# google-research/robopianist

Measured on AMD Instinct MI355X. Metric: env-steps/sec (whole node) at 4096 envs/GPU, higher is better.
Workload: dtype f64

## Files before the change

### include/rp_engine.h

```cpp
#ifndef RP_ENGINE_H
#define RP_ENGINE_H

#include <stddef.h>
#include <stdint.h>

#ifdef __cplusplus
extern "C" {
#endif

typedef struct rp_engine rp_engine;

typedef enum {
  RP_QPOS = 0,
  RP_QVEL = 1,
  RP_QACC_WARMSTART = 2,
  RP_CTRL = 3,
  RP_QFRC_APPLIED = 4,
  RP_ACT_FORCE = 5,
  RP_ACT_VELOCITY = 6,
  RP_SITE_XPOS = 7,
  RP_TIME = 8,
  RP_NCON = 9,
  RP_CONTACT_GEOMS = 10,
  RP_WARN_FLAGS = 11,
// ... 18 lines not shown
#define RP_WARN_SPLIT_FULL 64
#define RP_WARN_DENSE_FULL 32

int rp_create(const void* model_blob, size_t blob_bytes, int n_envs, int device_id,
              int precision, rp_engine** out);
int rp_destroy(rp_engine* e);

int rp_reset(rp_engine* e, const uint8_t* mask);

int rp_set(rp_engine* e, rp_field f, const void* src);
int rp_get(rp_engine* e, rp_field f, void* dst);

int rp_step(rp_engine* e, int n_substeps, uint32_t* key_trace);

int rp_forward(rp_engine* e);

int rp_step_masked(rp_engine* e, int n_substeps, uint32_t* key_trace, const uint8_t* reset_mask);

int rp_set_solver_limits(rp_engine* e, int max_newton_iter, int max_ls_iter);

int rp_set_solver_tolerance(rp_engine* e, double tolerance, double ls_tolerance);
int rp_set_mpr_tolerance(rp_engine* e, double tolerance, double polytope_tolerance);
int rp_set_lazy_position_stage(rp_engine* e, int on);
int rp_set_legacy_step(rp_engine* e, int on);
int rp_set_cost_ordered_launch(rp_engine* e, int on);
int rp_set_lean_solver(rp_engine* e, int on);

int rp_set_fused_substeps(rp_engine* e, int on);
int rp_get_fused_substeps(rp_engine* e);

int rp_set_split_position_stage(rp_engine* e, int on);
int rp_get_split_position_stage(rp_engine* e);

int rp_set_stream_slices(rp_engine* e, int n);
int rp_set_acc_sensors(rp_engine* e, int on);
int rp_sync(rp_engine* e);
int rp_get_stream(rp_engine* e, void** hip_stream);
int rp_set_stream(rp_engine* e, void* hip_stream);
int rp_field_ptr(rp_engine* e, rp_field f, void** ptr, size_t* bytes);
int rp_n_envs(const rp_engine* e);
int rp_dim(const rp_engine* e, const char* name);
int rp_kernel_time(rp_engine* e, double* avg_ms, int* n_launches);
int rp_solver_kernel_time(rp_engine* e, double* avg_ms, int* n_launches);
int rp_solver_kernel_envs(rp_engine* e, double* avg_envs);
int rp_solver_kernel_fused(rp_engine* e);
int rp_profile(rp_engine* e, long long* out, int n, int enable);
// ... 7 lines not shown
```

### robopianist_amd/csrc/rp_engine.hip

```cpp
#include "rp_kernels.hpp"
#include "rp_schedule.hpp"

#include <hip/hip_runtime.h>

#include <cmath>
#include <cstdio>
#include <cstdlib>
#include <cstring>
#include <map>
#include <mutex>
#include <string>
#include <vector>

#include "../../include/rp_engine.h"

namespace {

__global__ void rp_lead_mask_kernel(int* lead, const int* active, const unsigned char* valid, int lazy, const unsigned char* also, int n) {
  const int e = blockIdx.x * blockDim.x + threadIdx.x;
  if (e < n) lead[e] = (((active ? active[e] != 0 : true) && !(lazy && valid[e])) || (also && also[e])) ? 1 : 0;
}
__global__ void rp_mark_valid_kernel(unsigned char* valid, const int* active, const unsigned char* also, int n) {
  const int e = blockIdx.x * blockDim.x + threadIdx.x;
  if (e < n && (!active || active[e] != 0 || (also && also[e]))) valid[e] = 1;
}

#define RP_ORDER_BUCKETS 256
#define RP_ORDER_CLASSES 8
__global__ __launch_bounds__(512) void rp_order_kernel(int* order_all, const int* hdr, const int* active, int base, int n,
                                                       int* heavy_list, int* heavy_cnt, unsigned char* listed) {
  const int x = blockIdx.x;
  if (heavy_list) {
    for (int e = x + RP_ORDER_CLASSES * (int)threadIdx.x; e < n; e += RP_ORDER_CLASSES * blockDim.x) {
      const bool on = hdr[(base + e) * rpk::HDR_N + rpk::HDR_CLASS] != 1 && !(active && active[base + e] == 0);
      if (on) heavy_list[base + atomicAdd(heavy_cnt, 1)] = base + e;
      if (listed) listed[base + e] = on ? 1 : 0;
    }
  }
  if (!order_all) return;
  int* order = order_all + base;
  __shared__ int hist[RP_ORDER_BUCKETS];
  for (int i = threadIdx.x; i < RP_ORDER_BUCKETS; i += blockDim.x) hist[i] = 0;
  __syncthreads();
// ... 202 lines not shown
    if (!ev_pending[i]) return;
    if (wait) hipEventSynchronize(ev1[i]);
    else if (hipEventQuery(ev1[i]) != hipSuccess) return;
    float ms = 0;
    if (hipEventElapsedTime(&ms, ev0[i], ev1[i]) == hipSuccess) {
      kernel_ms += ms; kernel_launches++;
    }
    if (sv_envs[i] > 0 && hipEventElapsedTime(&ms, sv0[i], sv1[i]) == hipSuccess) {
      const int kd = sv_kind[i] & 1;
      solver_ms_k[kd] += ms; solver_launches_k[kd]++; solver_envs_k[kd] += sv_envs[i];
    }
    sv_envs[i] = 0;
    ev_pending[i] = false;
  }
  virtual int reset(const uint8_t* mask) = 0;
  virtual int set(rp_field f, const void* src) = 0;
  virtual int get(rp_field f, void* dst) = 0;
  virtual int step(int nsub, uint32_t* trace, int mode, const uint8_t* reset_mask = nullptr) = 0;
  virtual void limits(int newton, int ls) = 0;
  virtual void tolerances(double tol, double ls_tol) = 0;
  virtual void mpr_tolerances(double tol, double poly_tol) = 0;
  bool lazy_position = false;
  bool legacy_step = true;
  bool cost_order = false;
  int n_slices = 1;
  static const int kMaxSlices = kRpMaxSlices;
  hipStream_t xstream[kMaxSlices] = {};
  hipEvent_t ev_fork = nullptr, ev_join[kMaxSlices] = {};
  hipStream_t hstream[kMaxSlices] = {};
  hipEvent_t ev_hfork[kMaxSlices] = {}, ev_hjoin[kMaxSlices] = {};
  virtual int acc_sensors(int on) = 0;
  virtual int lean_solver(int on) = 0;
  virtual int fused_substeps(int on) = 0;
  virtual int fused_substeps_on() const = 0;
  virtual int split_position(int on) = 0;
  virtual int split_position_on() const = 0;
  virtual int field_ptr(rp_field f, void** p, size_t* bytes) = 0;
  bool own_stream = true;
  virtual int profile(long long* out, int n, int enable) = 0;
};

template <typename T>
struct Engine : EngineBase {
  RpModel<T> M{};
  RpState<T> S{};
  RpStage<T> B{};
// ... 242 lines not shown
    hipMemset(B.slots, 0xFF, sizeof(int) * E * rpk::SLOT_N);
    hipMemset(B.keyslot, 0xFF, sizeof(int) * E * (RPK_NKEYS / 4));
    S.key_trace = nullptr;
    S.prof = nullptr;
    d_active = dalloc<int>(E);
    S.active = nullptr;
    d_lead = dalloc<int>(E);
    d_order = dalloc<int>(E);
    {
      std::vector<int> id(E);
      for (size_t i = 0; i < E; i++) id[i] = (int)i;
      hipMemcpy(d_order, id.data(), E * sizeof(int), hipMemcpyHostToDevice);
    }
    S.cost_pos = dalloc<int>(E); S.cost_sol = dalloc<int>(E);
    d_heavy = dalloc<int>(E); d_heavy_cnt = dalloc<int>(2 * kMaxSlices);
    d_listed = dalloc<unsigned char>(E); S.listed = d_listed;
    d_heavy_peak = dalloc<int>(kMaxSlices + 1);
    if (hipHostMalloc((void**)&h_heavy_peak, sizeof(int) * (kMaxSlices + 1)) != hipSuccess) { (void)hipGetLastError(); h_heavy_peak = nullptr; }
    else { for (int i = 0; i < kMaxSlices; i++) h_heavy_peak[i] = -1; h_heavy_peak[kMaxSlices] = 0; }
    S.heavy_list = nullptr; S.heavy_cnt = nullptr; S.heavy_done = nullptr;
    S.qpos_prev = nullptr; S.qvel_prev = nullptr;
    d_valid = dalloc<unsigned char>(E);
    S.max_newton = M.iterations; S.max_ls = M.ls_iterations;
  }
  void read_switches() {
    {
      const char* sp = getenv("RP_SPLIT_POS");
      split_capable = sizeof(T) == 8 && !deep;
      split_mode = !split_capable ? 0 : (sp ? (sp[0] == '0' ? 0 : (sp[0] == '1' ? 1 : 2)) : 2);
    }
    {
      const char* le = getenv("RP_LEAN");
      lean = sizeof(T) == 8 && !deep && !(le && le[0] == '0');
      const char* dh = getenv("RP_DENSE_HANDS");
      dense_joint = (dh && dh[0] == '0') ? RPK_LEAN_JOINT : 0;
      S.lean = lean ? (1 | dense_joint) : 0;
      if (lean && le && atoi(le) > 1) S.lean = (atoi(le) & RPK_LEAN_CAP) | dense_joint;
    }
  }

  bool split_alloc_failed = false;
  bool ensure_split_buffers() {
    if (B.frames) return true;
    if (split_alloc_failed) return false;
    const size_t E = (size_t)nenv;
    const size_t mark = allocs.size();
    try {
      T* frames = dalloc<T>(E * RPK_NFRAME * 64);
      B.cand = dalloc<int>(E * RPK_NCAND * 2);
      B.ncand = dalloc<int>(E);
      B.cres = dalloc<T>(E * RPK_NRES * 12);
      B.cres_n = dalloc<int>(E * RPK_NCAND);
// ... 104 lines not shown
    if (newton > 0) S.max_newton = newton;
    if (ls > 0) S.max_ls = ls;
  }

  RpState<T> reset_state() const {
    RpState<T> sr = S;
    sr.sens_torque = sensors_on ? d_sens_torque : nullptr; sr.sens_touch = sensors_on ? d_sens_touch : nullptr;
    return sr;
  }
  RpState<T> heavy_state(const RpState<T>& ss, int sl, bool capturing) const {
    RpState<T> sh = ss;
    sh.heavy_list = d_heavy + ss.env_base; sh.heavy_cnt = d_heavy_cnt + 2 * sl; sh.heavy_done = d_heavy_cnt + 2 * sl + 1;
    sh.heavy_peak = capturing ? nullptr : d_heavy_peak + sl;
    return sh;
  }
  RpState<T> sensor_state(const RpState<T>& ss) const {
    RpState<T> sq = ss;
    sq.qpos = d_qpos_prev; sq.qvel = d_qvel_prev;
    sq.sens_torque = d_sens_torque; sq.sens_touch = d_sens_touch;
    sq.key_trace = nullptr; sq.prof = nullptr;
    return sq;
  }

  void launch_reset(const unsigned char* dmask) {
    hipLaunchKernelGGL(rp_reset_kernel<T>, dim3(nenv), dim3(64), 0, stream, reset_state(), d_qpos0, dmask, nv, nu, nsite, d_valid);
  }
  int reset(const uint8_t* mask) override {
    HIP_OK(hipSetDevice(device));
    const unsigned char* dmask = nullptr;
    if (mask) {
      if (is_device_ptr(mask)) dmask = mask;
      else {
        if (!d_mask) HIP_OK(hipMalloc((void**)&d_mask, (size_t)nenv));
        HIP_OK(hipMemcpyAsync(d_mask, mask, (size_t)nenv, hipMemcpyHostToDevice, stream));
        HIP_OK(hipStreamSynchronize(stream));
        dmask = d_mask;
      }
    }
    launch_reset(dmask);
    HIP_OK(hipGetLastError());
    return 0;
  }

  bool field(rp_field f, void** p, size_t* bytes, bool* writable) {
    size_t E = (size_t)nenv;
    *writable = false;
    switch (f) {
      case RP_QPOS: *p = S.qpos; *bytes = sizeof(T) * E * nv; *writable = true; return true;
      case RP_QVEL: *p = S.qvel; *bytes = sizeof(T) * E * nv; *writable = true; return true;
      case RP_QACC_WARMSTART: *p = S.warm; *bytes = sizeof(T) * E * nv; *writable = true; return true;
      case RP_CTRL: *p = S.ctrl; *bytes = sizeof(T) * E * nu; *writable = true; return true;
      case RP_QFRC_APPLIED: *p = S.qfrc_applied; *bytes = sizeof(T) * E * nv; *writable = true; return true;
      case RP_ACT_FORCE: *p = S.act_force; *bytes = sizeof(T) * E * nu; return true;
      case RP_ACT_VELOCITY: *p = S.act_vel; *bytes = sizeof(T) * E * nu; return true;
      case RP_SITE_XPOS: *p = S.site_xpos; *bytes = sizeof(T) * E * nsite * 3; return true;
      case RP_TIME: *p = S.time; *bytes = sizeof(T) * E; *writable = true; return true;
      case RP_NCON: *p = S.ncon; *bytes = sizeof(int) * E; return true;
      case RP_CONTACT_GEOMS: *p = S.contact_geoms; *bytes = sizeof(int) * E * RPK_NCOUT * 2; return true;
      case RP_WARN_FLAGS: *p = S.warn; *bytes = sizeof(int) * E; *writable = true; return true;
      case RP_SOLVER_ITER: *p = S.solver_iter; *bytes = sizeof(int) * E; return true;
      case RP_CONTACT_DIST: *p = S.contact_dist; *bytes = sizeof(T) * E * RPK_NCOUT; return true;
      case RP_ACTIVE: *p = d_active; *bytes = sizeof(int) * E; *writable = true; return true;
// ... 3 lines not shown
      case RP_DEBUG_HANDOVER_HDR: *p = B.hdr; *bytes = sizeof(int) * E * rpk::HDR_N; return true;
      case RP_SENSOR_TORQUE: if (!d_sens_torque) return false; *p = d_sens_torque; *bytes = sizeof(T) * E * nv; return true;
      case RP_SENSOR_TOUCH: if (!d_sens_touch) return false; *p = d_sens_touch; *bytes = sizeof(T) * E * nsite; return true;
    }
    return false;
  }
  int field_ptr(rp_field f, void** p, size_t* bytes) override {
    bool w;
    if (!field(f, p, bytes, &w)) return fail("rp_field_ptr: unknown field (sensor fields need rp_set_acc_sensors first)");
    if (f == RP_ACTIVE) S.active = d_active;
    return 0;
  }
  int set(rp_field f, const void* src) override {
    void* p; size_t nb; bool w;
    if (!field(f, &p, &nb, &w)) return fail("rp_set: unknown field");
    if (!w) return fail("rp_set: field is read-only");
    if (!src) { if (f == RP_ACTIVE) { S.active = nullptr; return 0; } return fail("rp_set: null source"); }
    HIP_OK(hipSetDevice(device));
    if (nb) {
      if (!is_device_ptr(src)) HIP_OK(hipStreamSynchronize(stream));
      HIP_OK(hipMemcpyAsync(p, src, nb, hipMemcpyDefault, stream));
    }
    if (f == RP_ACTIVE) S.active = d_active;
    if (f == RP_QPOS || f == RP_QVEL || f == RP_TREE_OFFSET) HIP_OK(hipMemsetAsync(d_valid, 0, (size_t)nenv, stream));
    return 0;
  }
  int get(rp_field f, void* dst) override {
    void* p; size_t nb; bool w;
    if (!field(f, &p, &nb, &w)) return fail("rp_get: unknown field");
    if (!dst) return fail("rp_get: null destination");
    HIP_OK(hipSetDevice(device));
    if (nb) HIP_OK(hipMemcpyAsync(dst, p, nb, hipMemcpyDefault, stream));
    if (!is_device_ptr(dst)) HIP_OK(hipStreamSynchronize(stream));
    return 0;
  }

  struct StepCtx {
    int nsub = 0, mode = 0;
    const uint8_t* reset_mask = nullptr;
    bool capturing = false, timeit = false, lead_masked = false;
    int slot = 0;
    RpStepInput in;
    RpStepPlan plan;
    int nsl = 1;
    RpState<T> s;
  };
  struct Slice {
// ... 152 lines not shown
      HIP_OK(hipEventRecord(ev_hjoin[sl], hs));
      RpState<T> sm_ = x.ss;
      sm_.skip_heavy = 1;
      emit_pos(c, x, sm_, k);
      HIP_OK(hipStreamWaitEvent(st, ev_hjoin[sl], 0));
    } else {
      emit_pos(c, x, x.ss, k);
    }
    return 0;
  }

  int finish(const StepCtx& c, uint32_t* trace, size_t trace_words) {
    HIP_OK(hipGetLastError());
    if (c.mode == 0) step_calls++;
    if (c.timeit) { HIP_OK(hipEventRecord(ev1[c.slot], stream)); ev_pending[c.slot] = true; }
    if (trace && c.mode == 0)
      HIP_OK(hipMemcpyAsync(trace, d_trace, trace_words * sizeof(uint32_t), hipMemcpyDefault, stream));
    return 0;
  }

  int step(int nsub, uint32_t* trace, int mode, const uint8_t* reset_mask = nullptr) override {
    HIP_OK(hipSetDevice(device));
    if (mode == 0 && nsub <= 0) return fail("rp_step: n_substeps must be positive");
    if (reset_mask) {
      if (!is_device_ptr(reset_mask)) return fail("rp_step_masked: the reset mask must be device memory");
      launch_reset(reset_mask);
    }
    StepCtx c;
    c.nsub = nsub; c.mode = mode; c.reset_mask = reset_mask;
    c.s = S;
    const size_t need = (size_t)nenv * (nsub > 0 ? nsub : 1) * 4;
    if (trace && mode == 0) {
      if (need > trace_cap) {
        if (d_trace) hipFree(d_trace);
        HIP_OK(hipMalloc((void**)&d_trace, need * sizeof(uint32_t)));
        trace_cap = need;
      }
      c.s.key_trace = d_trace;
    }
    RP_TRY(begin_timers(c));
    plan(c);
    if (cost_order && mode == 0) c.s.order = d_order;
    const bool lazy_now = lazy_position && legacy_step;
    c.s.stale_outputs = (!legacy_step && mode == 0) ? 1 : 0;
    c.lead_masked = (lazy_now || reset_mask) && mode == 0;
    if (c.lead_masked)
      hipLaunchKernelGGL(rp_lead_mask_kernel, dim3((nenv + 255) / 256), dim3(256), 0, stream, d_lead, c.s.active, d_valid, lazy_now ? 1 : 0, reset_mask, nenv);
    RP_TRY(fork_slices(c));
    for (int sl = 0; sl < c.nsl; sl++) {
      Slice x = slice_of(c, sl);
      RpState<T> lead = x.ss;
      lead.order = nullptr;
      if (c.lead_masked) lead.active = d_lead;
      emit_pos(c, x, lead, -1);
      if (mode != 0) continue;
      if (c.plan.fused_now && sizeof(T) == 8) { RP_TRY(emit_fused_slice(c, x)); continue; }
      for (int k = 0; k < nsub; k++) RP_TRY(emit_substep(c, x, k));
    }
    RP_TRY(join_slices(c));
    return finish(c, trace, need);
  }
};

EngineBase* E(rp_engine* e) { return reinterpret_cast<EngineBase*>(e); }

}

extern "C" {

const char* rp_last_error(void) { return g_err.c_str(); }

int rp_create(const void* model_blob, size_t blob_bytes, int n_envs, int device_id, int precision,
              rp_engine** out) {
  if (!out) return fail("rp_create: out is null");
  *out = nullptr;
  if (!model_blob || n_envs <= 0) return fail("rp_create: bad arguments");
  if (precision != 32 && precision != 64) return fail("rp_create: precision must be 32 or 64");
  Blob b;
  if (!b.init(model_blob, blob_bytes)) return fail("rp_create: not a model blob (bad magic)");
  if (!b.has("eng_nlink")) return fail("rp_create: blob lacks engine tables (eng_*)");
  int ndev = 0;
  if (hipGetDeviceCount(&ndev) != hipSuccess || ndev <= 0)
// ... 20 lines not shown
  if (r) { delete e; return r; }
  *out = reinterpret_cast<rp_engine*>(e);
  return 0;
}

int rp_destroy(rp_engine* e) {
  if (!e) return fail("rp_destroy: null engine");
  delete E(e);
  return 0;
}
int rp_reset(rp_engine* e, const uint8_t* mask) { return e ? E(e)->reset(mask) : fail("null engine"); }
int rp_set(rp_engine* e, rp_field f, const void* src) { return e ? E(e)->set(f, src) : fail("null engine"); }
int rp_get(rp_engine* e, rp_field f, void* dst) { return e ? E(e)->get(f, dst) : fail("null engine"); }
int rp_step(rp_engine* e, int n_substeps, uint32_t* key_trace) {
  return e ? E(e)->step(n_substeps, key_trace, 0) : fail("null engine");
}
int rp_forward(rp_engine* e) { return e ? E(e)->step(0, nullptr, 1) : fail("null engine"); }
int rp_step_masked(rp_engine* e, int n_substeps, uint32_t* key_trace, const uint8_t* reset_mask) {
  return e ? E(e)->step(n_substeps, key_trace, 0, reset_mask) : fail("null engine");
}
int rp_set_solver_limits(rp_engine* e, int max_newton_iter, int max_ls_iter) {
  if (!e) return fail("null engine");
  E(e)->limits(max_newton_iter, max_ls_iter);
  return 0;
}
int rp_profile(rp_engine* e, long long* out, int n, int enable) {
  return e ? E(e)->profile(out, n, enable) : fail("null engine");
}
int rp_set_mpr_tolerance(rp_engine* e, double tolerance, double polytope_tolerance) {
  if (!e) return fail("null engine");
  E(e)->mpr_tolerances(tolerance, polytope_tolerance);
  return 0;
}
int rp_set_solver_tolerance(rp_engine* e, double tolerance, double ls_tolerance) {
  if (!e) return fail("null engine");
  E(e)->tolerances(tolerance, ls_tolerance);
  return 0;
}
int rp_set_lazy_position_stage(rp_engine* e, int on) {
  if (!e) return fail("null engine");
  E(e)->lazy_position = on != 0;
  return 0;
}
int rp_set_legacy_step(rp_engine* e, int on) {
  if (!e) return fail("null engine");
  E(e)->legacy_step = on != 0;
  return 0;
}
int rp_set_acc_sensors(rp_engine* e, int on) { return e ? E(e)->acc_sensors(on) : fail("null engine"); }
int rp_set_lean_solver(rp_engine* e, int on) { return e ? E(e)->lean_solver(on) : fail("null engine"); }
int rp_set_fused_substeps(rp_engine* e, int on) { return e ? E(e)->fused_substeps(on) : fail("null engine"); }
int rp_get_fused_substeps(rp_engine* e) { return e ? E(e)->fused_substeps_on() : fail("null engine"); }
int rp_set_split_position_stage(rp_engine* e, int on) { return e ? E(e)->split_position(on) : fail("null engine"); }
int rp_get_split_position_stage(rp_engine* e) { return e ? E(e)->split_position_on() : fail("null engine"); }
int rp_set_stream_slices(rp_engine* e, int n) {
  if (!e) return fail("null engine");
  if (n != 0 && n != 1 && n != 2 && n != 3 && n != 4) return fail("rp_set_stream_slices: 0 (automatic), 1, 2, 3 or 4");
  E(e)->n_slices = n;
  return 0;
}
int rp_set_cost_ordered_launch(rp_engine* e, int on) {
  if (!e) return fail("null engine");
  E(e)->cost_order = on != 0;
  return 0;
}
int rp_sync(rp_engine* e) {
  if (!e) return fail("null engine");
  HIP_OK(hipSetDevice(E(e)->device));
  HIP_OK(hipStreamSynchronize(E(e)->stream));
  return 0;
}
int rp_set_stream(rp_engine* e, void* hip_stream) {
  if (!e) return fail("null engine");
  EngineBase* b = E(e);
  HIP_OK(hipSetDevice(b->device));
  HIP_OK(hipStreamSynchronize(b->stream));
  for (int i = 0; i < EngineBase::kRing; i++) b->harvest(i, true);
  if (b->own_stream && b->stream) HIP_OK(hipStreamDestroy(b->stream));
  b->stream = (hipStream_t)hip_stream;
  b->own_stream = false;
  return 0;
}
int rp_field_ptr(rp_engine* e, rp_field f, void** ptr, size_t* bytes) {
  if (!e || !ptr || !bytes) return fail("null argument");
  return E(e)->field_ptr(f, ptr, bytes);
}
// ... 55 lines not shown
```

### robopianist_amd/csrc/rp_kernels.hpp

```cpp
#pragma once
#include <type_traits>
#include "rp_model.hpp"
#include "rp_wave.hpp"
#include "rp_narrow.hpp"
#include "rp_collide.hpp"
#include "rp_dense.hpp"
#include "rp_solver2.hpp"
#include "rp_solver_full.hpp"

#define RPK_BOXBOX(rc_, bx_, pA_, mA_, sA_, pB_, mB_, sB_) [&]() -> int {                       \
    T a_[15], b_[15]; RawCon<T> o_[3];                                                          \
    _Pragma("unroll") for (int i_ = 0; i_ < 3; i_++) { a_[i_] = (pA_)[i_]; b_[i_] = (pB_)[i_]; a_[12 + i_] = (sA_)[i_]; b_[12 + i_] = (sB_)[i_]; } \
    _Pragma("unroll") for (int i_ = 0; i_ < 9; i_++) { a_[3 + i_] = (mA_)[i_]; b_[3 + i_] = (mB_)[i_]; }                     \
    const int n_ = box_box(o_, bx_, a_, a_ + 3, a_ + 12, b_, b_ + 3, b_ + 12);                  \
    (rc_)[0] = o_[0]; (rc_)[1] = o_[1]; (rc_)[2] = o_[2];                                       \
    return n_; }()
namespace rpk {
template <typename T, int MD>
struct Smem<T, 0, MD> : SmemShared<T> {
  T xpos[RPK_NLX(MD)][3];
  T xmat[RPK_NLX(MD)][9];
  T xaxis[RPK_NLX(MD)][3];
  T xanchor[RPK_NLX(MD)][3];
  union {
// ... 38 lines not shown
      unsigned short glist[RPK_GLIST];
      unsigned short klist[RPK_KLIST];
    };
  };
  union {
    T acc[RPK_NLX(MD)][10];
    struct {
      float gax[RPK_WAVE][4];
      float grr[RPK_WAVE];
      int clist[RPK_NCAND];
    };
  };
  T gpos[RPK_WAVE][3];
};
template <typename T, int MD>
struct Smem<T, 2, MD> : Smem<T, 0, MD> {
  T fext[RPK_NLX(MD)][6];
  T touch[RPK_WAVE];
};
}

template <typename T>
__global__ void rp_reset_kernel(RpState<T> S, const T* qpos0, const unsigned char* mask, int nv, int nu, int nsite,
                                unsigned char* stage_valid) {
  const int env = blockIdx.x;
  if (mask && !mask[env]) return;
  if (threadIdx.x == 0) stage_valid[env] = 0;
  for (int i = threadIdx.x; i < nv; i += blockDim.x) {
    S.qpos[(size_t)env * nv + i] = qpos0[i];
    S.qvel[(size_t)env * nv + i] = 0;
    S.warm[(size_t)env * nv + i] = 0;
    S.qfrc_applied[(size_t)env * nv + i] = 0;
  }
  for (int i = threadIdx.x; i < nu; i += blockDim.x) S.ctrl[(size_t)env * nu + i] = 0;
  if (threadIdx.x == 0) { S.time[env] = 0; S.warn[env] = 0; }
  if (S.sens_torque) for (int i = threadIdx.x; i < nv; i += blockDim.x) S.sens_torque[(size_t)env * nv + i] = 0;
  if (S.sens_touch) for (int i = threadIdx.x; i < nsite; i += blockDim.x) S.sens_touch[(size_t)env * nsite + i] = 0;
}

template <typename T, int MODE, int MD = RPK_MAXD, int MESH = 0, bool EXT = false, int PART = 0>
__device__ __forceinline__ void rp_position_body(const RpModel<T>& M, const RpState<T>& S, const RpStage<T>& B, const int substep,
                                                 const int nsub, const int env, void* ext, const int lane) {
  static_assert(MODE == 0 || MODE == 2, "position / velocity stage (0) or sensor stage (2)");
  using namespace rpk;
  using N = Num<T>;
  constexpr bool PB = MODE == 0 && PART == 2 && !EXT;
  constexpr bool PF = MODE == 0 && PART == 1 && !EXT;
  if constexpr (MODE == 0) {
    if constexpr (PART == 2) { if constexpr (!PB) { if (B.ncand[env] < 0) return; } }
    else if (S.skip_heavy && S.listed[env]) return;
  }
  const int env_active = S.active ? S.active[env] : 1;
  using SM_ = std::conditional_t<(MODE == 0 && PART == 1), SmemFront<T, MD>, Smem<T, MODE, MD>>;
  SM_& sm = rp_smem<SM_, EXT>(ext);
#ifdef RPK_POISON_LDS
  {
    unsigned* w_ = reinterpret_cast<unsigned*>(&sm);
    for (int i = threadIdx.x; i < (int)(sizeof(sm) / 4); i += 64) w_[i] = 0xFFF4DEADu;
// ... 1881 lines not shown
```

### robopianist_amd/csrc/rp_model.hpp

```cpp
#pragma once
#include <hip/hip_runtime.h>
#include <stdint.h>

#define RPK_WAVE 64
#define RPK_NC 64
#define RPK_NCOUT 64
#ifndef RPK_NCL
#define RPK_NCL 32
#endif
#ifndef RPK_NE
#define RPK_NE 640
#endif
#define RPK_EM0(lane_, con_, col_, cross_) ((lane_) | ((con_) << 6) | ((col_) << 12) | ((cross_) << 16))
#define RPK_EM1(base_, cnt_, rank_) ((base_) | ((cnt_) << 12) | ((rank_) << 18))
#define RPK_EM_LANE(m0_) ((m0_) & 63)
#define RPK_EM_CON(m0_) (((m0_) >> 6) & 63)
#define RPK_EM_COL(m0_) (((m0_) >> 12) & 15)
#define RPK_EM_CROSS(m0_) (((m0_) >> 16) & 1)
#define RPK_EM_BASE(m1_) ((m1_) & 4095)
#define RPK_EM_CNT(m1_) (((m1_) >> 12) & 63)
#define RPK_EM_RANK(m1_) (((m1_) >> 18) & 63)
#define RPK_NBOXF 32
#ifndef RPK_HMAX
#define RPK_HMAX 60
// ... 271 lines not shown
template <typename T>
struct RpStage {
  T* RM;
  T* lanef;
  int* lanei;
  int* hdr;
  T* entJ;
  int* entM;
  int* slots;
  int* keyslot;
  T* covf;
  int* covi;
  T* frames;
  int* cand;
  int* ncand;
  T* cres;
  int* cres_n;
  int* tlist;
  int* tcount;
  int tcount_off;
  size_t tstride;
  int* split_dropped;
};
```

### robopianist_amd/csrc/rp_schedule.hpp

```cpp
#pragma once

static const int kRpMaxSlices = 4;

struct RpStepInput {
  int nenv = 0;
  int mode = 0;
  int n_slices = 1;
  int fused = 2;
  bool fused_capable = false;
  int split_mode = 0;
  bool split_capable = false;
  bool split_dropped = false;
  bool capturing = false;
  bool lean = false, deep = false, graph = false;
  double heavy_est[kRpMaxSlices] = {8, 8, 8, 8};
  int last_nsl = 1;
  bool many_heavy = false;
};

struct RpStepPlan {
  int sched = 0;
  int nsl = 1;
  bool fused_now = false;
  bool split_wanted = false;
// ... 30 lines not shown
    else if (split_ok && !p.many_heavy) p.sched = 4;
    else p.sched = in.nenv >= kRpNoSlicesFrom ? 1 : 2;
    p.fused_now = p.sched == 3;
    want = p.sched == 2 ? 2 : (p.sched == 4 ? 3 : 1);
    sched4 = p.sched == 4;
  }
  p.split_wanted = in.split_capable && in.mode == 0 && (in.split_mode == 1 || sched4);
  p.nsl = (in.mode == 0 && want > 1 && in.nenv >= kRpSliceMinEnvs && !in.capturing && !p.fused_now) ? (want >= 4 ? 4 : want) : 1;
  p.companion_now = p.nsl <= 2;
  return p;
}

inline int rp_fused_report(const RpStepInput& in, int auto_mode) {
  return !in.fused_capable ? 0 : (in.fused == 1 ? 1 : (in.fused == 2 && in.n_slices == 0 ? (auto_mode == 3 ? 1 : 2) : 0));
}
inline int rp_split_report(const RpStepInput& in, int auto_mode) {
  return in.split_mode == 1 ? 1 : (in.split_mode == 2 && in.n_slices == 0 && in.nenv >= kRpFusedBelow && !in.split_dropped ? (auto_mode == 4 ? 1 : 2) : 0);
}

inline bool rp_heavy_pos_alongside(const RpStepInput& in, bool on_companion_stream, bool fp64, double est) {
  return on_companion_stream && !in.deep && !in.graph && fp64 && est >= kRpHeavyOn;
}

inline int rp_slice_bound(int nenv, int nsl, int sl) { return sl >= nsl ? nenv : (int)(((long long)nenv * sl / nsl + 7) / 8 * 8); }

inline int rp_order_threads_for(int cnt) {
  const int t = ((cnt / 16 + 63) / 64) * 64;
  return t < 64 ? 64 : (t > 512 ? 512 : t);
}

inline double rp_heavy_est_update(double est, int seen) { return seen > est ? seen : 0.9 * est + 0.1 * seen; }

inline int rp_heavy_grid(double est, int cnt, int max_grid) {
  int g = (int)(2.0 * est) + 2;
  g = g < 2 ? 2 : (g > max_grid ? max_grid : g);
  return cnt < g ? cnt : g;
}
```

### robopianist_amd/engine.py

```python

from __future__ import annotations

import ctypes
import os
from typing import Optional

import numpy as np

from robopianist_amd import _abi
from robopianist_amd.model import compile as mcompile
from robopianist_amd.model import engine_tables

_HERE = os.path.dirname(os.path.abspath(__file__))
LIB_PATH = os.environ.get("RP_ENGINE_LIB") or os.path.join(_HERE, "csrc", "librp_engine.so")

QPOS, QVEL, QACC_WARMSTART, CTRL, QFRC_APPLIED, ACT_FORCE, ACT_VELOCITY, SITE_XPOS, \
    TIME, NCON, CONTACT_GEOMS, WARN_FLAGS, SOLVER_ITER, CONTACT_DIST, TREE_OFFSET, ACTIVE, \
    SENSOR_TORQUE, SENSOR_TOUCH, ENV_COST, DEBUG_MASS_ROWS, DEBUG_HANDOVER_HDR = range(21)
MAX_CONTACTS = 64

WARN_BADSTATE = 1
WARN_CONTACT_FULL = 2
WARN_HESSIAN = 4
WARN_KEYSLOT_FULL = 8
WARN_WORK_FULL = 16
WARN_SPLIT_FULL = 64
WARN_DENSE_FULL = 32

EXPORTED_SYMBOLS = (
    "rp_create", "rp_destroy", "rp_reset", "rp_set", "rp_get", "rp_step", "rp_forward", "rp_step_masked",
    "rp_set_solver_limits", "rp_set_solver_tolerance", "rp_set_mpr_tolerance", "rp_set_lazy_position_stage", "rp_set_legacy_step", "rp_set_cost_ordered_launch", "rp_set_stream_slices", "rp_set_lean_solver", "rp_set_fused_substeps", "rp_get_fused_substeps", "rp_set_split_position_stage", "rp_get_split_position_stage", "rp_set_acc_sensors", "rp_sync", "rp_get_stream", "rp_set_stream", "rp_field_ptr",
    "rp_n_envs", "rp_dim",
    "rp_kernel_time", "rp_solver_kernel_time", "rp_solver_kernel_envs", "rp_solver_kernel_fused", "rp_profile", "rp_last_error",
)

_lib = None


class EngineError(RuntimeError):
    pass


def load_library(path: str = LIB_PATH):
    global _lib
    if _lib is not None:
        return _lib
    L = _abi.open_library(path, "engine", EngineError)
    L.rp_last_error.restype = ctypes.c_char_p
    L.rp_create.argtypes = [ctypes.c_char_p, ctypes.c_size_t, ctypes.c_int, ctypes.c_int,
                            ctypes.c_int, ctypes.POINTER(ctypes.c_void_p)]
    L.rp_destroy.argtypes = [ctypes.c_void_p]
    L.rp_reset.argtypes = [ctypes.c_void_p, ctypes.c_void_p]
    L.rp_set.argtypes = [ctypes.c_void_p, ctypes.c_int, ctypes.c_void_p]
    L.rp_get.argtypes = [ctypes.c_void_p, ctypes.c_int, ctypes.c_void_p]
    L.rp_step.argtypes = [ctypes.c_void_p, ctypes.c_int, ctypes.c_void_p]
    L.rp_forward.argtypes = [ctypes.c_void_p]
    L.rp_step_masked.argtypes = [ctypes.c_void_p, ctypes.c_int, ctypes.c_void_p, ctypes.c_void_p]
    L.rp_set_solver_limits.argtypes = [ctypes.c_void_p, ctypes.c_int, ctypes.c_int]
    L.rp_sync.argtypes = [ctypes.c_void_p]
    L.rp_set_solver_tolerance.argtypes = [ctypes.c_void_p, ctypes.c_double, ctypes.c_double]
    L.rp_set_mpr_tolerance.argtypes = [ctypes.c_void_p, ctypes.c_double, ctypes.c_double]
    L.rp_set_lazy_position_stage.argtypes = [ctypes.c_void_p, ctypes.c_int]
    L.rp_set_cost_ordered_launch.argtypes = [ctypes.c_void_p, ctypes.c_int]
    L.rp_set_acc_sensors.argtypes = [ctypes.c_void_p, ctypes.c_int]
    L.rp_set_stream_slices.argtypes = [ctypes.c_void_p, ctypes.c_int]
    L.rp_set_lean_solver.argtypes = [ctypes.c_void_p, ctypes.c_int]
    L.rp_set_legacy_step.argtypes = [ctypes.c_void_p, ctypes.c_int]
    L.rp_set_fused_substeps.argtypes = [ctypes.c_void_p, ctypes.c_int]
    L.rp_get_fused_substeps.argtypes = [ctypes.c_void_p]
    L.rp_set_split_position_stage.argtypes = [ctypes.c_void_p, ctypes.c_int]
    L.rp_get_split_position_stage.argtypes = [ctypes.c_void_p]
    L.rp_get_stream.argtypes = [ctypes.c_void_p, ctypes.POINTER(ctypes.c_void_p)]
    L.rp_n_envs.argtypes = [ctypes.c_void_p]
    L.rp_dim.argtypes = [ctypes.c_void_p, ctypes.c_char_p]
    L.rp_kernel_time.argtypes = [ctypes.c_void_p, ctypes.POINTER(ctypes.c_double),
                                 ctypes.POINTER(ctypes.c_int)]
    L.rp_solver_kernel_time.argtypes = [ctypes.c_void_p, ctypes.POINTER(ctypes.c_double),
                                        ctypes.POINTER(ctypes.c_int)]
    L.rp_solver_kernel_envs.argtypes = [ctypes.c_void_p, ctypes.POINTER(ctypes.c_double)]
    L.rp_solver_kernel_fused.argtypes = [ctypes.c_void_p]
    L.rp_profile.argtypes = [ctypes.c_void_p, ctypes.c_void_p, ctypes.c_int, ctypes.c_int]
    L.rp_set_stream.argtypes = [ctypes.c_void_p, ctypes.c_void_p]
    L.rp_field_ptr.argtypes = [ctypes.c_void_p, ctypes.c_int, ctypes.POINTER(ctypes.c_void_p),
                               ctypes.POINTER(ctypes.c_size_t)]
    _lib = L
# ... 117 lines not shown
        if out is None:
            out = np.empty(self.field_shape(f), self.field_dtype(f))
        self._check(self._L.rp_get(self._h, f, _ptr(out)))
        return out

    def step(self, n_substeps: int = 1, key_trace=None):
        self._check(self._L.rp_step(self._h, int(n_substeps), _ptr(key_trace)))

    def forward(self):
        self._check(self._L.rp_forward(self._h))

    def step_masked(self, n_substeps: int, key_trace, reset_mask):
        self._check(self._L.rp_step_masked(self._h, int(n_substeps), _ptr(key_trace), _ptr(reset_mask)))

    def sync(self):
        self._check(self._L.rp_sync(self._h))

    def set_solver_limits(self, max_newton_iter=0, max_ls_iter=0):
        self._check(self._L.rp_set_solver_limits(self._h, max_newton_iter, max_ls_iter))

    def set_lazy_position_stage(self, on: bool = True):
        self._check(self._L.rp_set_lazy_position_stage(self._h, int(bool(on))))

    def set_acc_sensors(self, on: bool = True):
        self._check(self._L.rp_set_acc_sensors(self._h, int(bool(on))))

    def set_stream_slices(self, n: int = 0):
        self._check(self._L.rp_set_stream_slices(self._h, int(n)))

    def set_legacy_step(self, on: bool = True):
        self._check(self._L.rp_set_legacy_step(self._h, int(bool(on))))

    def set_lean_solver(self, on=True):
        self._check(self._L.rp_set_lean_solver(self._h, int(on)))

    def set_fused_substeps(self, on=True):
        self._check(self._L.rp_set_fused_substeps(self._h, 2 if on == "auto" else int(on)))

    @property
    def fused_substeps(self) -> bool:
        return self._L.rp_get_fused_substeps(self._h) == 1

    def set_split_position_stage(self, on=True):
        self._check(self._L.rp_set_split_position_stage(self._h, 2 if on == "auto" else int(on)))

    @property
# ... 89 lines not shown
```

### robopianist_amd/suite/physics.py

```python

from __future__ import annotations

import os

import torch

from robopianist_amd import engine as eng


class TorchPhysics:
    def __init__(self, scene_info, n_envs: int, device_id: int = 0, precision: int = 64):
        if not torch.cuda.is_available():
            raise eng.EngineError(
                "No HIP device visible: the batched engine has no CPU fallback.")
        self.scene = scene_info
        self.model = scene_info.model
        self.n_envs = n_envs
        self.device = torch.device("cuda", device_id)
        self.dtype = torch.float32 if precision == 32 else torch.float64
        self.engine = eng.BatchedPhysics(self.model, scene_info.key_joint_ids, n_envs,
                                         device_id=device_id, precision=precision)
        with torch.cuda.device(self.device):
            self._stream = torch.cuda.current_stream(self.device)
            self.engine.set_stream(self._stream.cuda_stream)
        e = self.engine
        self.qpos = e.view(eng.QPOS)
        self.qvel = e.view(eng.QVEL)
        self.act_force = e.view(eng.ACT_FORCE)
        self.act_vel = e.view(eng.ACT_VELOCITY)
        self.site_xpos_eng = e.view(eng.SITE_XPOS)
        self.contact_geoms = e.view(eng.CONTACT_GEOMS)
        self.time = e.view(eng.TIME)
        self.warn = e.view(eng.WARN_FLAGS)
        self._ctrl = e.view(eng.CTRL)
        self._qfrc_applied = e.view(eng.QFRC_APPLIED)
        self._tree_offset = e.view(eng.TREE_OFFSET) if e.ntree else None
        self._active = e.view(eng.ACTIVE)
        self._active.fill_(1)
        e.set_lazy_position_stage(True)
        e.set_cost_ordered_launch(os.environ.get("RP_COST_ORDER", "1") != "0")
        e.set_stream_slices(int(os.environ.get("RP_STREAM_SLICES", "0")))
        from robopianist_amd.model import engine_tables
        t = engine_tables.build_engine_tables(self.model, scene_info.key_joint_ids)
        self._site_modelid = {int(s): i for i, s in enumerate(t["eng_site_modelid"])}
        self._site_index_cache = {}
        self.timestep = float(self.model.opt_timestep)

    def enable_acc_sensors(self):
        if getattr(self, "sens_torque", None) is None:
            self.engine.set_acc_sensors(True)
            self.sens_torque = self.engine.view(eng.SENSOR_TORQUE)
            self.sens_touch = self.engine.view(eng.SENSOR_TOUCH)

    def site_touch(self, model_site_ids):
        self.enable_acc_sensors()
        idx = torch.as_tensor([self._site_modelid[int(s)] for s in model_site_ids], dtype=torch.long, device=self.device)
        return self.sens_touch.index_select(1, idx)

    def renderer(self, colorize_fingertips: bool = False):
        key = bool(colorize_fingertips)
        cache = self.__dict__.setdefault("_renderers", {})
        if key not in cache:
# ... 40 lines not shown
    def refresh(self):
        """Views alias engine memory; nothing to copy."""

    def site_xpos(self, model_site_ids):
        key = tuple(int(s) for s in model_site_ids)
        idx = self._site_index_cache.get(key)
        if idx is None:
            idx = torch.as_tensor([self._site_modelid[s] for s in key], dtype=torch.long, device=self.device)
            self._site_index_cache[key] = idx
        return self.site_xpos_eng.index_select(1, idx)

    @property
    def ctrl(self):
        return self._ctrl

    def set_ctrl(self, ctrl: torch.Tensor):
        self._ctrl.copy_(ctrl)

    def set_qfrc_applied(self, f):
        self._qfrc_applied.copy_(torch.as_tensor(f, dtype=self.dtype, device=self.device)
                                 .expand(self.n_envs, self.model.nv))

    def set_tree_offset(self, off):
        self._tree_offset.copy_(torch.as_tensor(off, dtype=self.dtype, device=self.device))

    @property
    def active_mask(self):
        return self._active

    def set_active(self, mask: torch.Tensor):
        self._active.copy_(mask)

    _STATE_FIELDS = ("qpos", "qvel", "qacc_warmstart", "ctrl", "qfrc_applied", "time", "tree_offset")

    def _state_views(self):
        if not hasattr(self, "_warm"):
            self._warm = self.engine.view(eng.QACC_WARMSTART)
        v = {"qpos": self.qpos, "qvel": self.qvel, "qacc_warmstart": self._warm, "ctrl": self._ctrl,
             "qfrc_applied": self._qfrc_applied, "time": self.time}
        if self._tree_offset is not None:
            v["tree_offset"] = self._tree_offset
        return v

    def state_dict(self):
        return {k: v.detach().clone() for k, v in self._state_views().items()}

    def state_views(self):
        return dict(self._state_views())

    def load_state_dict(self, sd):
        views = self._state_views()
        for k, v in views.items():
            v.copy_(sd[k].to(device=self.device, dtype=v.dtype))
        self._active.fill_(1)
        self.engine.forward()

    def reset(self, mask=None):
        if mask is not None:
            mask = mask.to(torch.uint8).contiguous()
            self._reset_mask = mask
        self.engine.reset(mask)

    def forward(self):
        self.engine.forward()

    def step(self, n_substeps: int, key_trace=None):
        self.engine.step(n_substeps, key_trace)

    def step_masked(self, n_substeps: int, key_trace, reset_mask):
        self._reset_mask = reset_mask
        self.engine.step_masked(n_substeps, key_trace, reset_mask)
```

Baseline: 747,000.

## Snapshot reset-state position stage and copy it into reset envs, skipping lead pass

Builds a single-env snapshot of the position-stage handover buffers and outputs from qpos0. Reset envs then copy that snapshot in the reset kernel and are marked stage-valid instead of rerunning the position stage. When all envs are known valid under the lazy position stage, the lead-mask kernel and lead position pass are skipped entirely. This needs state tracking for option changes, tree-offset writes and graph capture to invalidate the snapshot, and it adds complexity and correctness risk.

```diff
diff --git a/include/rp_engine.h b/include/rp_engine.h
--- a/include/rp_engine.h
+++ b/include/rp_engine.h
@@ -64,6 +64,7 @@
 int rp_set_solver_tolerance(rp_engine* e, double tolerance, double ls_tolerance);
 int rp_set_mpr_tolerance(rp_engine* e, double tolerance, double polytope_tolerance);
 int rp_set_lazy_position_stage(rp_engine* e, int on);
+int rp_set_reset_snapshot(rp_engine* e, int on);
 int rp_set_legacy_step(rp_engine* e, int on);
 int rp_set_cost_ordered_launch(rp_engine* e, int on);
 int rp_set_lean_solver(rp_engine* e, int on);
diff --git a/robopianist_amd/csrc/rp_engine.hip b/robopianist_amd/csrc/rp_engine.hip
--- a/robopianist_amd/csrc/rp_engine.hip
+++ b/robopianist_amd/csrc/rp_engine.hip
@@ -16,9 +16,9 @@
 
 namespace {
 
-__global__ void rp_lead_mask_kernel(int* lead, const int* active, const unsigned char* valid, int lazy, const unsigned char* also, int n) {
+__global__ void rp_lead_mask_kernel(int* lead, const int* active, const unsigned char* valid, int lazy, const unsigned char* also, int also_lazy, int n) {
   const int e = blockIdx.x * blockDim.x + threadIdx.x;
-  if (e < n) lead[e] = (((active ? active[e] != 0 : true) && !(lazy && valid[e])) || (also && also[e])) ? 1 : 0;
+  if (e < n) lead[e] = (((active ? active[e] != 0 : true) && !(lazy && valid[e])) || (also && also[e] && !(also_lazy && valid[e]))) ? 1 : 0;
 }
 __global__ void rp_mark_valid_kernel(unsigned char* valid, const int* active, const unsigned char* also, int n) {
   const int e = blockIdx.x * blockDim.x + threadIdx.x;
@@ -267,6 +267,10 @@
   virtual void mpr_tolerances(double tol, double poly_tol) = 0;
   bool lazy_position = false;
   bool legacy_step = true;
+  RpSnapshotState snap;
+  void option_changed() { rp_snapshot_on_option(snap); }
+  virtual int snapshot_flag_changed() = 0;
+  virtual int reset_snapshot(int on) = 0;
   bool cost_order = false;
   int n_slices = 1;
   static const int kMaxSlices = kRpMaxSlices;
@@ -555,12 +559,70 @@
     S.qpos_prev = nullptr; S.qvel_prev = nullptr;
     d_valid = dalloc<unsigned char>(E);
     S.max_newton = M.iterations; S.max_ls = M.ls_iterations;
+    alloc_snapshot();
+  }
+  RpSnapshot<T> P{};
+  int* d_snap_ok = nullptr;
+  void alloc_snapshot() {
+    RpState<T>& s = P.S;
+    s = RpState<T>{};
+    s.nenv = 1;
+    s.qpos = dalloc<T>(nv); s.qvel = dalloc<T>(nv); s.warm = dalloc<T>(nv);
+    s.ctrl = dalloc<T>(nu); s.qfrc_applied = dalloc<T>(nv); s.time = dalloc<T>(1);
+    s.tree_offset = dalloc<T>((ntree ? ntree : 1) * 3);
+    s.act_force = dalloc<T>(nu); s.act_vel = dalloc<T>(nu);
+    s.site_xpos = dalloc<T>((nsite ? nsite : 1) * 3);
+    s.contact_dist = dalloc<T>(RPK_NCOUT);
+    s.ncon = dalloc<int>(1); s.contact_geoms = dalloc<int>(RPK_NCOUT * 2);
+    s.warn = dalloc<int>(1); s.solver_iter = dalloc<int>(1);
+    s.cost_pos = dalloc<int>(1); s.cost_sol = dalloc<int>(1);
+    RpStage<T>& b = P.B;
+    b = RpStage<T>{};
+    P.md = md();
+#define X(buf, per_env, live) b.buf = dalloc<std::remove_pointer_t<decltype(b.buf)>>(per_env);
+    { const int md = P.md; RPK_SNAPSHOT_HANDOVER(X) }
+#undef X
+    d_snap_valid = dalloc<unsigned char>(1);
+    d_snap_ok = dalloc<int>(1);
+    P.ok = d_snap_ok;
+  }
+  void build_snapshot() {
+    RpState<T> s = P.S;
+    s.max_newton = S.max_newton; s.max_ls = S.max_ls; s.lean = S.lean;
+    RpSnapshot<T> none{};
+    hipLaunchKernelGGL(rp_reset_kernel<T>, dim3(1), dim3(64), 0, stream, s, d_qpos0, (const unsigned char*)nullptr, nv, nu, nsite, d_snap_valid, P.B, none);
+    launch_stage<T, 0>(variant, 1, stream, M, s, P.B, -1, 1);
+    snap_built = true;
+    rp_snapshot_on_built(snap);
+    snapshot_flag_changed();
+  }
+  unsigned char* d_snap_valid = nullptr;
+  bool snap_built = false;
+  int reset_snapshot(int on) override {
+    HIP_OK(hipSetDevice(device));
+    snap.enabled = on != 0;
+    option_changed();
+    if (!on) {
+      HIP_OK(hipMemsetAsync(d_valid, 0, (size_t)nenv, stream));
+      rp_snapshot_on_state_write(snap, false, stream_capturing());
+    }
+    return snapshot_flag_changed();
+  }
+  int snapshot_flag_changed() override {
+    if (!d_snap_ok || !snap_built) return 0;
+    HIP_OK(hipSetDevice(device));
+    HIP_OK(hipMemsetAsync(d_snap_ok, (rp_snapshot_flag(snap) && snap_built) ? 1 : 0, 1, stream));
+    return 0;
   }
   void read_switches() {
     {
       const char* sp = getenv("RP_SPLIT_POS");
       split_capable = sizeof(T) == 8 && !deep;
       split_mode = !split_capable ? 0 : (sp ? (sp[0] == '0' ? 0 : (sp[0] == '1' ? 1 : 2)) : 2);
+    }
+    {
+      const char* rs = getenv("RP_RESET_SNAPSHOT");
+      snap.enabled = rs && rs[0] != '0';
     }
     {
       const char* le = getenv("RP_LEAN");
@@ -711,8 +773,20 @@
     return sq;
   }
 
-  void launch_reset(const unsigned char* dmask) {
-    hipLaunchKernelGGL(rp_reset_kernel<T>, dim3(nenv), dim3(64), 0, stream, reset_state(), d_qpos0, dmask, nv, nu, nsite, d_valid);
+  bool launch_reset(const unsigned char* dmask, bool capturing, bool lead_follows) {
+    const RpSnapshotUse use = rp_snapshot_use(snap, capturing);
+    if (use == kRpSnapBuild) build_snapshot();
+    const bool used = use != kRpSnapNone;
+    RpSnapshot<T> p = P;
+    if (!used) p.ok = nullptr;
+    hipLaunchKernelGGL(rp_reset_kernel<T>, dim3(nenv), dim3(used ? 256 : 64), 0, stream, reset_state(), d_qpos0, dmask, nv, nu, nsite, d_valid, B, p);
+    rp_snapshot_on_reset(snap, used, dmask == nullptr, lead_follows, capturing);
+    return used;
+  }
+  bool stream_capturing() const {
+    hipStreamCaptureStatus cap = hipStreamCaptureStatusNone;
+    (void)hipStreamIsCapturing(stream, &cap);
+    return cap != hipStreamCaptureStatusNone;
   }
   int reset(const uint8_t* mask) override {
     HIP_OK(hipSetDevice(device));
@@ -726,7 +800,7 @@
         dmask = d_mask;
       }
     }
-    launch_reset(dmask);
+    launch_reset(dmask, stream_capturing(), false);
     HIP_OK(hipGetLastError());
     return 0;
   }
@@ -776,7 +850,11 @@
       HIP_OK(hipMemcpyAsync(p, src, nb, hipMemcpyDefault, stream));
     }
     if (f == RP_ACTIVE) S.active = d_active;
-    if (f == RP_QPOS || f == RP_QVEL || f == RP_TREE_OFFSET) HIP_OK(hipMemsetAsync(d_valid, 0, (size_t)nenv, stream));
+    if (f == RP_QPOS || f == RP_QVEL || f == RP_TREE_OFFSET) {
+      HIP_OK(hipMemsetAsync(d_valid, 0, (size_t)nenv, stream));
+      rp_snapshot_on_state_write(snap, f == RP_TREE_OFFSET, stream_capturing());
+      if (f == RP_TREE_OFFSET) RP_TRY(snapshot_flag_changed());
+    }
     return 0;
   }
   int get(rp_field f, void* dst) override {
@@ -975,9 +1053,10 @@
   int step(int nsub, uint32_t* trace, int mode, const uint8_t* reset_mask = nullptr) override {
     HIP_OK(hipSetDevice(device));
     if (mode == 0 && nsub <= 0) return fail("rp_step: n_substeps must be positive");
+    bool snap_used = false;
     if (reset_mask) {
       if (!is_device_ptr(reset_mask)) return fail("rp_step_masked: the reset mask must be device memory");
-      launch_reset(reset_mask);
+      snap_used = launch_reset(reset_mask, stream_capturing(), true);
     }
     StepCtx c;
     c.nsub = nsub; c.mode = mode; c.reset_mask = reset_mask;
@@ -997,20 +1076,24 @@
     const bool lazy_now = lazy_position && legacy_step;
     c.s.stale_outputs = (!legacy_step && mode == 0) ? 1 : 0;
     c.lead_masked = (lazy_now || reset_mask) && mode == 0;
-    if (c.lead_masked)
-      hipLaunchKernelGGL(rp_lead_mask_kernel, dim3((nenv + 255) / 256), dim3(256), 0, stream, d_lead, c.s.active, d_valid, lazy_now ? 1 : 0, reset_mask, nenv);
+    const bool no_lead = rp_lead_skippable(snap, mode, lazy_now, c.capturing, reset_mask != nullptr, snap_used);
+    if (c.lead_masked && !no_lead)
+      hipLaunchKernelGGL(rp_lead_mask_kernel, dim3((nenv + 255) / 256), dim3(256), 0, stream, d_lead, c.s.active, d_valid, lazy_now ? 1 : 0, reset_mask, snap_used ? 1 : 0, nenv);
     RP_TRY(fork_slices(c));
     for (int sl = 0; sl < c.nsl; sl++) {
       Slice x = slice_of(c, sl);
-      RpState<T> lead = x.ss;
-      lead.order = nullptr;
-      if (c.lead_masked) lead.active = d_lead;
-      emit_pos(c, x, lead, -1);
+      if (!no_lead) {
+        RpState<T> lead = x.ss;
+        lead.order = nullptr;
+        if (c.lead_masked) lead.active = d_lead;
+        emit_pos(c, x, lead, -1);
+      }
       if (mode != 0) continue;
       if (c.plan.fused_now && sizeof(T) == 8) { RP_TRY(emit_fused_slice(c, x)); continue; }
       for (int k = 0; k < nsub; k++) RP_TRY(emit_substep(c, x, k));
     }
     RP_TRY(join_slices(c));
+    rp_snapshot_on_step_done(snap, c.s.active != nullptr, c.capturing);
     return finish(c, trace, need);
   }
 };
@@ -1077,6 +1160,7 @@
 int rp_set_solver_limits(rp_engine* e, int max_newton_iter, int max_ls_iter) {
   if (!e) return fail("null engine");
   E(e)->limits(max_newton_iter, max_ls_iter);
+  E(e)->option_changed();
   return 0;
 }
 int rp_profile(rp_engine* e, long long* out, int n, int enable) {
@@ -1085,38 +1169,49 @@
 int rp_set_mpr_tolerance(rp_engine* e, double tolerance, double polytope_tolerance) {
   if (!e) return fail("null engine");
   E(e)->mpr_tolerances(tolerance, polytope_tolerance);
+  E(e)->option_changed();
   return 0;
 }
 int rp_set_solver_tolerance(rp_engine* e, double tolerance, double ls_tolerance) {
   if (!e) return fail("null engine");
   E(e)->tolerances(tolerance, ls_tolerance);
+  E(e)->option_changed();
   return 0;
 }
 int rp_set_lazy_position_stage(rp_engine* e, int on) {
   if (!e) return fail("null engine");
   E(e)->lazy_position = on != 0;
-  return 0;
+  E(e)->option_changed();
+  return 0;
+}
+int rp_set_reset_snapshot(rp_engine* e, int on) {
+  if (!e) return fail("null engine");
+  return E(e)->reset_snapshot(on);
 }
 int rp_set_legacy_step(rp_engine* e, int on) {
   if (!e) return fail("null engine");
   E(e)->legacy_step = on != 0;
-  return 0;
-}
-int rp_set_acc_sensors(rp_engine* e, int on) { return e ? E(e)->acc_sensors(on) : fail("null engine"); }
-int rp_set_lean_solver(rp_engine* e, int on) { return e ? E(e)->lean_solver(on) : fail("null engine"); }
-int rp_set_fused_substeps(rp_engine* e, int on) { return e ? E(e)->fused_substeps(on) : fail("null engine"); }
+  E(e)->option_changed();
+  E(e)->snap.legacy_step = on != 0;
+  return E(e)->snapshot_flag_changed();
+}
+int rp_set_acc_sensors(rp_engine* e, int on) { if (e) E(e)->option_changed(); return e ? E(e)->acc_sensors(on) : fail("null engine"); }
+int rp_set_lean_solver(rp_engine* e, int on) { if (e) E(e)->option_changed(); return e ? E(e)->lean_solver(on) : fail("null engine"); }
+int rp_set_fused_substeps(rp_engine* e, int on) { if (e) E(e)->option_changed(); return e ? E(e)->fused_substeps(on) : fail("null engine"); }
 int rp_get_fused_substeps(rp_engine* e) { return e ? E(e)->fused_substeps_on() : fail("null engine"); }
-int rp_set_split_position_stage(rp_engine* e, int on) { return e ? E(e)->split_position(on) : fail("null engine"); }
+int rp_set_split_position_stage(rp_engine* e, int on) { if (e) E(e)->option_changed(); return e ? E(e)->split_position(on) : fail("null engine"); }
 int rp_get_split_position_stage(rp_engine* e) { return e ? E(e)->split_position_on() : fail("null engine"); }
 int rp_set_stream_slices(rp_engine* e, int n) {
   if (!e) return fail("null engine");
   if (n != 0 && n != 1 && n != 2 && n != 3 && n != 4) return fail("rp_set_stream_slices: 0 (automatic), 1, 2, 3 or 4");
   E(e)->n_slices = n;
+  E(e)->option_changed();
   return 0;
 }
 int rp_set_cost_ordered_launch(rp_engine* e, int on) {
   if (!e) return fail("null engine");
   E(e)->cost_order = on != 0;
+  E(e)->option_changed();
   return 0;
 }
 int rp_sync(rp_engine* e) {
diff --git a/robopianist_amd/csrc/rp_kernels.hpp b/robopianist_amd/csrc/rp_kernels.hpp
--- a/robopianist_amd/csrc/rp_kernels.hpp
+++ b/robopianist_amd/csrc/rp_kernels.hpp
@@ -84,10 +84,21 @@
 
 template <typename T>
 __global__ void rp_reset_kernel(RpState<T> S, const T* qpos0, const unsigned char* mask, int nv, int nu, int nsite,
-                                unsigned char* stage_valid) {
+                                unsigned char* stage_valid, RpStage<T> B, RpSnapshot<T> P) {
   const int env = blockIdx.x;
   if (mask && !mask[env]) return;
-  if (threadIdx.x == 0) stage_valid[env] = 0;
+  const bool snap = P.ok && *P.ok == 1;
+  if (snap) {
+    const int md = P.md;
+    const int* h = P.B.hdr;
+#define X(buf, per_env, live) rp_copy_wide(B.buf + (size_t)env * (per_env), P.B.buf, (live));
+    RPK_SNAPSHOT_HANDOVER(X)
+#undef X
+#define X(arr, per_env) if (S.arr) for (int i = threadIdx.x; i < (per_env); i += blockDim.x) S.arr[(size_t)env * (per_env) + i] = P.S.arr[i];
+    RPK_SNAPSHOT_OUTPUTS(X)
+#undef X
+  }
+  if (threadIdx.x == 0) stage_valid[env] = snap ? 1 : 0;
   for (int i = threadIdx.x; i < nv; i += blockDim.x) {
     S.qpos[(size_t)env * nv + i] = qpos0[i];
     S.qvel[(size_t)env * nv + i] = 0;
@@ -95,7 +106,7 @@
     S.qfrc_applied[(size_t)env * nv + i] = 0;
   }
   for (int i = threadIdx.x; i < nu; i += blockDim.x) S.ctrl[(size_t)env * nu + i] = 0;
-  if (threadIdx.x == 0) { S.time[env] = 0; S.warn[env] = 0; }
+  if (threadIdx.x == 0) { S.time[env] = 0; if (!snap) S.warn[env] = 0; }
   if (S.sens_torque) for (int i = threadIdx.x; i < nv; i += blockDim.x) S.sens_torque[(size_t)env * nv + i] = 0;
   if (S.sens_touch) for (int i = threadIdx.x; i < nsite; i += blockDim.x) S.sens_touch[(size_t)env * nsite + i] = 0;
 }
diff --git a/robopianist_amd/csrc/rp_model.hpp b/robopianist_amd/csrc/rp_model.hpp
--- a/robopianist_amd/csrc/rp_model.hpp
+++ b/robopianist_amd/csrc/rp_model.hpp
@@ -317,3 +317,39 @@
   size_t tstride;
   int* split_dropped;
 };
+
+#define RPK_SNAPSHOT_HANDOVER(X)                                                                          \
+  X(RM, RPK_NLX(md) * (md + 1), RPK_NLX(md) * (md + 1))                                                   \
+  X(lanef, RPK_NLF * 64, RPK_NLF * 64)                                                                    \
+  X(lanei, RPK_NLI * 64, RPK_NLI * 64)                                                                    \
+  X(hdr, rpk::HDR_N, rpk::HDR_RESUME)                                                                     \
+  X(entJ, RpCaps<T>::NE * 3, rp_clampi(h[rpk::HDR_NENT], 0, RpCaps<T>::NE) * 3)                           \
+  X(entM, RpCaps<T>::NE * 2, rp_clampi(h[rpk::HDR_NENT], 0, RpCaps<T>::NE) * 2)                           \
+  X(slots, rpk::SLOT_N, rpk::SLOT_N)                                                                      \
+  X(keyslot, RPK_NKEYS / 4, RPK_NKEYS / 4)                                                                \
+  X(covf, (RPK_NC - RPK_NCL) * 12, rp_clampi(h[rpk::HDR_NCON] - RPK_NCL, 0, RPK_NC - RPK_NCL) * 12)        \
+  X(covi, (RPK_NC - RPK_NCL) * 4, rp_clampi(h[rpk::HDR_NCON] - RPK_NCL, 0, RPK_NC - RPK_NCL) * 4)
+#define RPK_SNAPSHOT_OUTPUTS(X)                                                                           \
+  X(act_vel, nu) X(site_xpos, nsite * 3) X(contact_geoms, RPK_NCOUT * 2) X(contact_dist, RPK_NCOUT)        \
+  X(ncon, 1) X(cost_pos, 1) X(warn, 1)
+__host__ __device__ __forceinline__ int rp_clampi(int v, int lo, int hi) { return v < lo ? lo : (v > hi ? hi : v); }
+template <typename T>
+struct RpSnapshot {
+  RpState<T> S;
+  RpStage<T> B;
+  const int* ok;
+  int md;
+};
+template <typename U>
+__device__ __forceinline__ void rp_copy_wide(U* __restrict__ dst, const U* __restrict__ src, int n) {
+  static_assert(16 % sizeof(U) == 0, "element size");
+  constexpr int W = 16 / sizeof(U);
+  const int t = (int)threadIdx.x, nt = (int)blockDim.x;
+  if ((((size_t)dst | (size_t)src) & 15) == 0) {
+    const int nw = n / W;
+    for (int i = t; i < nw; i += nt) ((int4*)dst)[i] = ((const int4*)src)[i];
+    for (int i = nw * W + t; i < n; i += nt) dst[i] = src[i];
+  } else {
+    for (int i = t; i < n; i += nt) dst[i] = src[i];
+  }
+}
diff --git a/robopianist_amd/csrc/rp_schedule.hpp b/robopianist_amd/csrc/rp_schedule.hpp
--- a/robopianist_amd/csrc/rp_schedule.hpp
+++ b/robopianist_amd/csrc/rp_schedule.hpp
@@ -76,6 +76,40 @@
   return on_companion_stream && !in.deep && !in.graph && fp64 && est >= kRpHeavyOn;
 }
 
+struct RpSnapshotState {
+  bool enabled = true;
+  bool fresh = false;
+  bool tree_offset_set = false;
+  bool legacy_step = true;
+  bool all_valid = false;
+  bool poisoned = false;
+};
+enum RpSnapshotUse { kRpSnapNone = 0, kRpSnapUse = 1, kRpSnapBuild = 2 };
+inline RpSnapshotUse rp_snapshot_use(const RpSnapshotState& s, bool capturing) {
+  if (!s.enabled || s.tree_offset_set || !s.legacy_step) return kRpSnapNone;
+  if (s.fresh) return kRpSnapUse;
+  return capturing ? kRpSnapNone : kRpSnapBuild;
+}
+inline bool rp_snapshot_flag(const RpSnapshotState& s) { return s.enabled && !s.tree_offset_set && s.legacy_step; }
+inline void rp_snapshot_on_option(RpSnapshotState& s) { s.fresh = false; }
+inline void rp_snapshot_on_built(RpSnapshotState& s) { s.fresh = true; }
+inline void rp_snapshot_on_state_write(RpSnapshotState& s, bool tree_offset, bool capturing) {
+  s.all_valid = false;
+  if (tree_offset) s.tree_offset_set = true;
+  if (capturing) s.poisoned = true;
+}
+inline void rp_snapshot_on_reset(RpSnapshotState& s, bool used, bool whole_batch, bool lead_follows, bool capturing) {
+  if (capturing) { s.poisoned = true; s.all_valid = false; return; }
+  if (used) s.all_valid = s.all_valid || whole_batch;
+  else if (!lead_follows) s.all_valid = false;
+}
+inline void rp_snapshot_on_step_done(RpSnapshotState& s, bool active_mask, bool capturing) {
+  if (!capturing && !active_mask && !s.poisoned) s.all_valid = true;
+}
+inline bool rp_lead_skippable(const RpSnapshotState& s, int mode, bool lazy_now, bool capturing, bool has_reset, bool snap_used) {
+  return s.enabled && mode == 0 && lazy_now && !capturing && !s.poisoned && s.all_valid && (!has_reset || snap_used);
+}
+
 inline int rp_slice_bound(int nenv, int nsl, int sl) { return sl >= nsl ? nenv : (int)(((long long)nenv * sl / nsl + 7) / 8 * 8); }
 
 inline int rp_order_threads_for(int cnt) {
diff --git a/robopianist_amd/engine.py b/robopianist_amd/engine.py
--- a/robopianist_amd/engine.py
+++ b/robopianist_amd/engine.py
@@ -29,7 +29,7 @@
 
 EXPORTED_SYMBOLS = (
     "rp_create", "rp_destroy", "rp_reset", "rp_set", "rp_get", "rp_step", "rp_forward", "rp_step_masked",
-    "rp_set_solver_limits", "rp_set_solver_tolerance", "rp_set_mpr_tolerance", "rp_set_lazy_position_stage", "rp_set_legacy_step", "rp_set_cost_ordered_launch", "rp_set_stream_slices", "rp_set_lean_solver", "rp_set_fused_substeps", "rp_get_fused_substeps", "rp_set_split_position_stage", "rp_get_split_position_stage", "rp_set_acc_sensors", "rp_sync", "rp_get_stream", "rp_set_stream", "rp_field_ptr",
+    "rp_set_solver_limits", "rp_set_solver_tolerance", "rp_set_mpr_tolerance", "rp_set_lazy_position_stage", "rp_set_reset_snapshot", "rp_set_legacy_step", "rp_set_cost_ordered_launch", "rp_set_stream_slices", "rp_set_lean_solver", "rp_set_fused_substeps", "rp_get_fused_substeps", "rp_set_split_position_stage", "rp_get_split_position_stage", "rp_set_acc_sensors", "rp_sync", "rp_get_stream", "rp_set_stream", "rp_field_ptr",
     "rp_n_envs", "rp_dim",
     "rp_kernel_time", "rp_solver_kernel_time", "rp_solver_kernel_envs", "rp_solver_kernel_fused", "rp_profile", "rp_last_error",
 )
@@ -61,6 +61,7 @@
     L.rp_set_solver_tolerance.argtypes = [ctypes.c_void_p, ctypes.c_double, ctypes.c_double]
     L.rp_set_mpr_tolerance.argtypes = [ctypes.c_void_p, ctypes.c_double, ctypes.c_double]
     L.rp_set_lazy_position_stage.argtypes = [ctypes.c_void_p, ctypes.c_int]
+    L.rp_set_reset_snapshot.argtypes = [ctypes.c_void_p, ctypes.c_int]
     L.rp_set_cost_ordered_launch.argtypes = [ctypes.c_void_p, ctypes.c_int]
     L.rp_set_acc_sensors.argtypes = [ctypes.c_void_p, ctypes.c_int]
     L.rp_set_stream_slices.argtypes = [ctypes.c_void_p, ctypes.c_int]
@@ -224,6 +225,9 @@
     def set_lazy_position_stage(self, on: bool = True):
         self._check(self._L.rp_set_lazy_position_stage(self._h, int(bool(on))))
 
+    def set_reset_snapshot(self, on: bool = True):
+        self._check(self._L.rp_set_reset_snapshot(self._h, int(bool(on))))
+
     def set_acc_sensors(self, on: bool = True):
         self._check(self._L.rp_set_acc_sensors(self._h, int(bool(on))))
 
diff --git a/robopianist_amd/suite/physics.py b/robopianist_amd/suite/physics.py
--- a/robopianist_amd/suite/physics.py
+++ b/robopianist_amd/suite/physics.py
@@ -38,6 +38,8 @@
         self._active = e.view(eng.ACTIVE)
         self._active.fill_(1)
         e.set_lazy_position_stage(True)
+        if os.environ.get("RP_RESET_SNAPSHOT", "1") != "0":
+            e.set_reset_snapshot(True)
         e.set_cost_ordered_launch(os.environ.get("RP_COST_ORDER", "1") != "0")
         e.set_stream_slices(int(os.environ.get("RP_STREAM_SLICES", "0")))
         from robopianist_amd.model import engine_tables
@@ -124,7 +126,9 @@
                                  .expand(self.n_envs, self.model.nv))
 
     def set_tree_offset(self, off):
-        self._tree_offset.copy_(torch.as_tensor(off, dtype=self.dtype, device=self.device))
+        off = torch.as_tensor(off, dtype=self.dtype, device=self.device).expand(self._tree_offset.shape).contiguous()
+        self._tree_offset_src = off
+        self.engine.set(eng.TREE_OFFSET, off)
 
     @property
     def active_mask(self):
@@ -148,12 +152,20 @@
         return {k: v.detach().clone() for k, v in self._state_views().items()}
 
     def state_views(self):
-        return dict(self._state_views())
+        views = dict(self._state_views())
+        if "tree_offset" in views:
+            self.engine.set_reset_snapshot(False)
+        return views
 
     def load_state_dict(self, sd):
         views = self._state_views()
         for k, v in views.items():
-            v.copy_(sd[k].to(device=self.device, dtype=v.dtype))
+            src = sd[k].to(device=self.device, dtype=v.dtype)
+            if k == "tree_offset":
+                if not torch.equal(src.reshape(v.shape), v):
+                    self.set_tree_offset(src.reshape(v.shape))
+                continue
+            v.copy_(src)
         self._active.fill_(1)
         self.engine.forward()
 
```

Result: faster. 757,300 (median of 6 runs) (+1.4%).
